# qiutang98/chord

Measured on AMD Instinct MI355X. Metric: Gtri/s into 4K 64-bit visbuffer, higher is better.
Workload: dtype f32+u64; 1 GPU; street_4k_hzb; scene_triangles_lod0=2799616, objects=352, hzb=True, cull=flat, parallelism=single

## Files before the change

chord_amd/csrc/device_layer.h:

```cpp
#pragma once

#include <hip/hip_runtime.h>
#include <cstddef>

#include <string>
#include <vector>

#include "chordvis.h"

#ifndef RASTER_PROFILE
#define RASTER_PROFILE 0
#endif
#ifndef RASTER_ABLATION
#define RASTER_ABLATION 0
#endif
#define CHORD_DEBUG_PROFILE_BITS (16u | 512u)
#define CHORD_DEBUG_ABLATION_BITS (1u | 2u | 32u | 64u | 128u | 256u | 1024u | 2048u | 4096u | 8192u | 16384u | 1048576u | 2097152u)

namespace chord {


struct DPrim {
    float    posMin[3]; uint32_t meshletBase;
    float    posMax[3]; uint32_t groupBase;
// ... 121 lines not shown
struct TriRecC {
    int32_t  X0, Y0;
    int16_t  dX1, dY1, dX2, dY2;
    float    d[3];
    uint32_t payload;
};
#define CHORD_REC_WIDE 0x80000000u
#define CHORD_REC_BLOCK 0xC0000000u
#define CHORD_REC_INDEX_MASK 0x3FFFFFFFu
#define CHORD_REC_MASKED 0xA0000000u
#define CHORD_REC_WIDE_INDEX 0x1FFFFFFFu
#define CHORD_BLOCK_WIN 16
struct ClipTri { uint32_t objectId, meshletId, slot, tri; };

#define CHORD_LIST_SHARDS 64u
#define CHORD_SHARD_STRIDE 16u
struct DeviceCounters {
    uint32_t triCount[CHORD_LIST_SHARDS * CHORD_SHARD_STRIDE];
    uint32_t triCountC[CHORD_LIST_SHARDS * CHORD_SHARD_STRIDE];
    uint32_t clipTriCount[2];
    uint32_t largeCount[2][CHORD_LIST_SHARDS * CHORD_SHARD_STRIDE];
    uint32_t overflow;
    uint32_t binPoolCount[2];
    uint32_t pad;
    uint32_t blockGranules[CHORD_LIST_SHARDS * CHORD_SHARD_STRIDE];
    uint32_t pad3[10];
    unsigned long long trisInstanceCulled, trisHzbVisible0, trisHzbVisible1, pad2;
};

#define CHORD_BIN_CHUNK_SHIFT 10
#define CHORD_BIN_CHUNK (1u << CHORD_BIN_CHUNK_SHIFT)
#define CHORD_BIN_MAX_CHUNKS_DEFAULT 240u
#define CHORD_BIN_MAX_CHUNKS_LIMIT 3072u
#define CHORD_TILE_MAX_SLICES 64u
#define CHORD_BIN_CHUNK_INVALID 0xFFFFFFFFu
#define CHORD_TILE_SLICE_SHIFT 11
#define CHORD_HOT_TILES 32u
#ifndef CHORD_TILE_SHIFT
#define CHORD_TILE_SHIFT 6
#endif
#define CHORD_TILE (1 << CHORD_TILE_SHIFT)
#define CHORD_MAX_TILES ((4096u >> CHORD_TILE_SHIFT) * (4096u >> CHORD_TILE_SHIFT))
#if CHORD_TILE_SHIFT == 6
#define CHORD_TILECOUNT_STRIDE 16u
#ifndef CHORD_BIN_CAP
#define CHORD_BIN_CAP 16384u
#endif
#else
#define CHORD_TILECOUNT_STRIDE 4u
#define CHORD_BIN_CAP 8192u
#endif
static_assert(CHORD_BIN_CAP <= (1u << 20), "tile x bin capacity is formed with a 24-bit multiply in 32 bits (bin_put)");
struct FrameState {
    DeviceCounters counters;
    uint32_t listCounts[8];
    uint32_t tileCount[2 * CHORD_MAX_TILES * CHORD_TILECOUNT_STRIDE];
};

static_assert(offsetof(FrameState, counters.trisInstanceCulled) % 64 == 0 && offsetof(FrameState, listCounts) == offsetof(FrameState, counters.trisInstanceCulled) + 32 &&
              offsetof(FrameState, tileCount) == offsetof(FrameState, listCounts) + 32, "triangle totals + list counts: one 64-byte line (frame_cull_fused_kernel)");

struct CmdList {
    uint32_t*     count = nullptr;
    ChordDrawCmd* cmds = nullptr;
    uint32_t      capacity = 0;
    ChordCountAndCmd handle() const { return ChordCountAndCmd{count, cmds, capacity}; }
};

struct HzbBuffers {
    ChordHZBDesc desc{};
    uint16_t* minTexels = nullptr;
    uint16_t* maxTexels = nullptr;
    uint32_t* validRange = nullptr;
    bool valid = false;
    bool uploaded = false;
    ChordHZB handle() const { return ChordHZB{desc, minTexels, maxTexels, validRange}; }
};

enum StampTag { S_FRAME_BEGIN = 0, S_CLEAR, S_CULL, S_HZBCULL, S_R_CLUSTER, S_R_CLIP, S_R_CHUNK, S_STAGE0_END,
                S_HZB0, S_STAGE1_END, S_HZBF, S_OTHER,
                S_EXCH_HZB, S_EXCH_VIS,
                S_EXCH_CULL,
                S_EXCH_FINAL };

}

struct ChordCtx {
    int device = 0;
    hipStream_t stream = nullptr;
    bool ownStream = false;
    std::string lastError;
    int numCUs = 256;

    bool sceneLoaded = false;
    uint32_t objectCount = 0, primCount = 0, materialCount = 0;
    uint32_t meshletCount = 0, groupCount = 0;
    uint32_t groupInstances = 0;
    uint32_t cmdCapacity = 0;
    uint64_t instTriangles = 0;
    chord::DPrim* dPrims = nullptr;
    chord::DGroup* dGroups = nullptr;
    chord::DMeshlet* dMeshlets = nullptr;
    uint32_t* dGroupIndices = nullptr;
    uint32_t* dMeshletData = nullptr;
    float* dPositions = nullptr;
    chord::DObjStatic* dObjStatic = nullptr;
// ... 195 lines not shown
```

chord_amd/csrc/kernels_raster.hip:

```cpp

#include "device_layer.h"
#include "device_math.h"

#include <algorithm>
#include <cstdlib>
#include <cstring>
#include <type_traits>

namespace chord {

#define GUARD_BAND 1024.0f
#define LDS_VERTS 256
#define TILE CHORD_TILE
#define TILE_SHIFT CHORD_TILE_SHIFT
#define TPITCH (TILE + 1)
#define SMALL_AREA 256
#define TC_STRIDE CHORD_TILECOUNT_STRIDE
#define TC_BLOCKS 1u
#define TC_TICKET 2u
#ifndef CHORD_MASKED_FUSED
#define CHORD_MASKED_FUSED 1
#endif
#define TC_MASKED 3u

struct RasterParams {
    const uint32_t* count; const ChordDrawCmd* cmds;
    uint32_t cmdCap;
    uint32_t* leftCount; ChordDrawCmd* leftCmds;
    const DObjFrame* objFrame; const DObjStatic* objStatic;
    const DMeshlet* meshlets; const uint32_t* meshletData; const float* positions;
    const DMaterial* materials; const uint8_t* texAlpha; const float* texcoords;
    unsigned long long* vis;
    float* depthOut;
    float W, H; int32_t Wi, Hi;
    ShardInfo shard;
    TriRec* tris; uint32_t triCap;
    TriRecC* trisC; uint32_t triCapC;
    uint32_t* tileCount; uint32_t* tileBins; uint32_t binCap; uint32_t tilesX, tilesY;
    uint32_t* binPool; uint32_t binPoolChunks; uint32_t* binPoolCount;
    unsigned long long* binChunkTab; uint32_t binStamp; uint32_t binMaxChunks;
    unsigned long long* blockPool; uint32_t blockCap;
    uint32_t blockForce;
    ClipTri* clipTris; uint32_t clipTriCap; uint32_t pass;
    uint32_t* largeList; uint32_t largeCap;
    DeviceCounters* counters;
    uint2* tileOrder;
    unsigned long long* tileSlabs;
    uint32_t hzbFused;
    ChordHZBDesc hzbDesc;
    uint16_t* hzbMinA;
    uint16_t* hzbMinB; uint16_t* hzbMaxB;
    uint16_t* hzbExA;
    uint16_t* hzbExB;
    uint32_t* tileRange;
    unsigned long long* tileClocks;
    unsigned long long* tilePhase;
    uint32_t depthOnly, depthClamp;
    float biasConst, biasSlope;
    uint32_t clearTiles;
    uint32_t* binHint;
    uint32_t* countHint;
    uint32_t slotHot;
    uint32_t* hotTiles;
    uint32_t tileSlots;
    uint32_t tileSplitMin, tileSliceLen;
    uint2* tileOrderNext;
    uint32_t orderAll;
    uint32_t orderKept;
    uint32_t* heavyHint;
    uint32_t debug;
};
#define ABL(p, flag) (RASTER_ABLATION && ((p).debug & (flag)) != 0u)
#define DBG_NO_PIXELS   1u
#define DBG_NO_BIN      2u
#define DBG_TILE_CLOCKS 16u
#define DBG_NO_OUT      128u
#define DBG_NO_HZB      256u
#define DBG_SETUP_CLOCKS 512u
#define DBG_NO_VIS_STORE 1024u
#define DBG_NO_SPLIT    2048u
#define DBG_NO_TINY     32u
#define DBG_TILE_EXIT   64u
#define DBG_NO_ENTRY    8192u
#define DBG_NO_BATCH    16384u
#define DBG_NO_UNITS    4096u
#define DBG_SKIP_LIGHT  1048576u
#define DBG_SKIP_HEAVY  2097152u

template <typename T>
__device__ __forceinline__ T scalar_load(const T* ptr)
{
    return *reinterpret_cast<const __attribute__((address_space(4))) T*>(reinterpret_cast<uintptr_t>(ptr));
}
__device__ __forceinline__ const RasterParams* kernel_args()
{
    unsigned long long kp = (unsigned long long)__builtin_amdgcn_kernarg_segment_ptr();
    asm volatile("" : "+s"(kp));
    return reinterpret_cast<const RasterParams*>(kp);
}

__device__ __forceinline__ uint32_t mbcnt64(unsigned long long m) { return __builtin_amdgcn_mbcnt_hi((uint32_t)(m >> 32), __builtin_amdgcn_mbcnt_lo((uint32_t)m, 0u)); }
__device__ __forceinline__ int32_t bcast(int32_t v, int src) { return __builtin_amdgcn_readlane(v, src); }
__device__ __forceinline__ uint32_t bcast(uint32_t v, int src) { return (uint32_t)__builtin_amdgcn_readlane((int)v, src); }
__device__ __forceinline__ float bcast(float v, int src) { return __int_as_float(__builtin_amdgcn_readlane(__float_as_int(v), src)); }

__device__ __forceinline__ bool owns_tile(const ShardInfo& s, int32_t tx, int32_t ty)
{
    if (s.ranks <= 1) return true;
    return shard_owns_tile(s, (uint32_t)tx, (uint32_t)ty);
}
__device__ __forceinline__ bool owns_rect(const ShardInfo& s, int32_t px0, int32_t py0, int32_t px1, int32_t py1)
{
    if (s.ranks <= 1) return true;
    return shard_owns_any_tile(s, (uint32_t)px0 >> TILE_SHIFT, (uint32_t)py0 >> TILE_SHIFT, (uint32_t)px1 >> TILE_SHIFT, (uint32_t)py1 >> TILE_SHIFT);
}

__device__ __forceinline__ bool in_fast_volume_xy(const f4& h)
{
    return h.w > 0.0f && (GUARD_BAND * h.w + h.x) >= 0.0f && (GUARD_BAND * h.w - h.x) >= 0.0f &&
           (GUARD_BAND * h.w + h.y) >= 0.0f && (GUARD_BAND * h.w - h.y) >= 0.0f;
}

// ... 71 lines not shown
    const float dzdx = ((float)(double)(a1 * 256) * invA) * e1 + ((float)(double)(a2 * 256) * invA) * e2;
    const float dzdy = ((float)(double)(b1 * 256) * invA) * e1 + ((float)(double)(b2 * 256) * invA) * e2;
    const float m = fmaxf(fabsf(dzdx), fabsf(dzdy));
    const float mz = fmaxf(fabsf(d[0]), fmaxf(fabsf(d[1]), fabsf(d[2])));
    const int32_t e = (int32_t)((__float_as_uint(mz) >> 23) & 0xFFu) - 23;
    const float r = (e > 0 && e < 255) ? __uint_as_float((uint32_t)e << 23) : 0.0f;
    return biasSlope * m + biasConst * r;
}

__device__ __forceinline__ void tri_setup_from_compact(TriSetup& ts, const TriRecC& r, int32_t Wi, int32_t Hi)
{
    ts.X[0] = r.X0; ts.Y[0] = r.Y0;
    ts.X[1] = r.X0 + r.dX1; ts.Y[1] = r.Y0 + r.dY1;
    ts.X[2] = r.X0 + r.dX2; ts.Y[2] = r.Y0 + r.dY2;
    ts.payload = r.payload;
    const int32_t area2 = (int32_t)r.dX1 * (int32_t)r.dY2 - (int32_t)r.dX2 * (int32_t)r.dY1;
    ts.s = area2 < 0 ? -1 : 1;
    ts.invA = 1.0f / (float)(area2 < 0 ? -area2 : area2);
    ts.d0 = r.d[0]; ts.e1 = r.d[1] - r.d[0]; ts.e2 = r.d[2] - r.d[0];
    const int32_t minX = min(ts.X[0], min(ts.X[1], ts.X[2])), maxX = max(ts.X[0], max(ts.X[1], ts.X[2]));
    const int32_t minY = min(ts.Y[0], min(ts.Y[1], ts.Y[2])), maxY = max(ts.Y[0], max(ts.Y[1], ts.Y[2]));
    ts.px0 = max(0, (minX + 127) >> 8);
    ts.py0 = max(0, (minY + 127) >> 8);
    ts.px1 = min(Wi - 1, (maxX - 128) >> 8);
    ts.py1 = min(Hi - 1, (maxY - 128) >> 8);
    ts.area = 0;
}

__device__ __forceinline__ void tri_setup_from_record(TriSetup& ts, const TriRec& r, int32_t Wi, int32_t Hi)
{
#pragma unroll
    for (int i = 0; i < 3; i++) { ts.X[i] = r.X[i]; ts.Y[i] = r.Y[i]; }
    ts.payload = r.payload;
    ts.s = (r.twoSided & 2u) ? -1 : 1;
    ts.invA = __uint_as_float(r.pad);
    ts.d0 = r.d[0]; ts.e1 = r.d[1] - r.d[0]; ts.e2 = r.d[2] - r.d[0];
    const int32_t minX = min(ts.X[0], min(ts.X[1], ts.X[2])), maxX = max(ts.X[0], max(ts.X[1], ts.X[2]));
    const int32_t minY = min(ts.Y[0], min(ts.Y[1], ts.Y[2])), maxY = max(ts.Y[0], max(ts.Y[1], ts.Y[2]));
    ts.px0 = max(0, (minX + 127) >> 8);
    ts.py0 = max(0, (minY + 127) >> 8);
    ts.px1 = min(Wi - 1, (maxX - 128) >> 8);
    ts.py1 = min(Hi - 1, (maxY - 128) >> 8);
    ts.area = 0;
}



struct RecordEmitParams {
    DeviceCounters* counters; ClipTri* clipTris; uint32_t clipTriCap; uint32_t pass;
    TriRec* tris; uint32_t triCap; TriRecC* trisC; uint32_t triCapC; uint32_t* largeList; uint32_t largeCap;
    uint32_t* tileCount; uint32_t* tileBins; uint32_t binCap; uint32_t tilesX;
    uint32_t* binPool; uint32_t binPoolChunks; uint32_t* binPoolCount;
    unsigned long long* binChunkTab; uint32_t binStamp; uint32_t binMaxChunks;
    ShardInfo shard;
};
__device__ __forceinline__ RecordEmitParams load_record_emit_params()
{
    const RasterParams* q = kernel_args();
    RecordEmitParams e;
    e.counters = scalar_load(&q->counters); e.clipTris = scalar_load(&q->clipTris); e.clipTriCap = scalar_load(&q->clipTriCap); e.pass = scalar_load(&q->pass);
    e.tris = scalar_load(&q->tris); e.triCap = scalar_load(&q->triCap); e.trisC = scalar_load(&q->trisC); e.triCapC = scalar_load(&q->triCapC);
    e.largeList = scalar_load(&q->largeList); e.largeCap = scalar_load(&q->largeCap);
    e.tileCount = scalar_load(&q->tileCount); e.tileBins = scalar_load(&q->tileBins); e.binCap = scalar_load(&q->binCap); e.tilesX = scalar_load(&q->tilesX);
    e.binPool = scalar_load(&q->binPool); e.binPoolChunks = scalar_load(&q->binPoolChunks); e.binPoolCount = scalar_load(&q->binPoolCount);
    e.binChunkTab = scalar_load(&q->binChunkTab); e.binStamp = scalar_load(&q->binStamp); e.binMaxChunks = scalar_load(&q->binMaxChunks);
    e.shard.ranks = scalar_load(&q->shard.ranks); e.shard.rank = scalar_load(&q->shard.rank); e.shard.slotsPerRank = 0u; e.shard.tilesX = 0u;
    e.shard.ownedRows = scalar_load(&q->shard.ownedRows); e.shard.tileSlot = nullptr;
    return e;
}

struct BinElect { int leader; uint32_t rank, group; };

__device__ __forceinline__ BinElect wave_bin_elect(bool has, uint32_t tile, uint32_t lane)
{
    BinElect e; e.leader = 0; e.rank = 0; e.group = 0;
    unsigned long long todo = __ballot(has);
    const unsigned long long lt = (1ull << lane) - 1ull;
    while (todo) {
        const int l = __ffsll((long long)todo) - 1;
        const uint32_t k = bcast(tile, l);
        const unsigned long long same = __ballot(has && tile == k);
        if (has && tile == k) { e.leader = l; e.rank = (uint32_t)__popcll(same & lt); e.group = (uint32_t)__popcll(same); }
        todo &= ~same;
    }
    return e;
}

__device__ __forceinline__ uint32_t bin_capacity(const RasterParams& p) { return p.binCap + p.binMaxChunks * CHORD_BIN_CHUNK; }

template <class P>
__device__ __forceinline__ void bin_alloc(const P& p, uint32_t tile, uint32_t slot)
{
#ifdef EXP_NO_CHUNKS
    return;
#endif
    if (slot < p.binCap) return;
    const uint32_t o = slot - p.binCap, j = o >> CHORD_BIN_CHUNK_SHIFT;
    if (j >= p.binMaxChunks || (o & (CHORD_BIN_CHUNK - 1u)) != 0u) return;
    uint32_t id = atomicAdd(p.binPoolCount, 1u);
    if (id >= p.binPoolChunks) { id = CHORD_BIN_CHUNK_INVALID; atomicOr(&p.counters->overflow, 1u); }
    __hip_atomic_store(p.binChunkTab + (__umul24(tile, p.binMaxChunks) + j), ((unsigned long long)p.binStamp << 32) | id,
                       __ATOMIC_RELAXED, __HIP_MEMORY_SCOPE_AGENT);
}

template <class P>
__device__ __forceinline__ void bin_put(const P& p, uint32_t tile, uint32_t slot, uint32_t gi)
{
#ifdef EXP_NO_CHUNKS
    slot &= p.binCap - 1u;
#endif
    if (slot < p.binCap) { p.tileBins[__umul24(tile, p.binCap) + slot] = gi; return; }
    const uint32_t o = slot - p.binCap, j = o >> CHORD_BIN_CHUNK_SHIFT;
    if (j >= p.binMaxChunks) { atomicOr(&p.counters->overflow, 1u); return; }
    const unsigned long long* ent = p.binChunkTab + (__umul24(tile, p.binMaxChunks) + j);
    const unsigned long long stamp = (unsigned long long)p.binStamp << 32;
    unsigned long long e = 0;
    uint32_t spins = 0;
    for (;;) {
        e = __hip_atomic_load(ent, __ATOMIC_RELAXED, __HIP_MEMORY_SCOPE_AGENT);
        if ((e & 0xFFFFFFFF00000000ull) == stamp) break;
        if (++spins > (1u << 20)) { atomicOr(&p.counters->overflow, 4u); return; }
        __builtin_amdgcn_s_sleep(4);
    }
    const uint32_t id = (uint32_t)e;
    if (id != CHORD_BIN_CHUNK_INVALID) p.binPool[((size_t)id << CHORD_BIN_CHUNK_SHIFT) + (o & (CHORD_BIN_CHUNK - 1u))] = gi;
}

__device__ __forceinline__ void bin_store(const RasterParams& p, uint32_t tile, uint32_t slot, uint32_t gi)
{
    bin_alloc(p, tile, slot);
    bin_put(p, tile, slot, gi);
}

struct BinTicket {
    uint32_t tileA[4], tileB[4], slotA[4], slotB[4];
    uint32_t has;
    uint32_t eA[4], eB[4];
};

template <class P>
__device__ __forceinline__ void wave_bin_issue(const P& p, bool emitA, const TriSetup& tsA, bool emitB, const TriSetup& tsB,
                                               uint32_t lane, BinTicket& k, const bool masked = false)
{
    auto tile_of = [&](const TriSetup& ts, int r, bool emit, uint32_t& tile) -> bool {
        const int32_t tx0 = ts.px0 >> TILE_SHIFT, tx1 = ts.px1 >> TILE_SHIFT, ty0 = ts.py0 >> TILE_SHIFT, ty1 = ts.py1 >> TILE_SHIFT;
// ... 474 lines not shown
                const uint32_t li = ebaseW + wSlots * (uint32_t)__popcll(ewA & lt);
                if (li + wSlots <= e.triCap) {
                    giA = listShard * e.triCap + li; write_record(&e.tris[giA], tsA, dA, twoSided, masked);
                    if (MASKED && masked) setup_emit_mask_ext(p, &e.tris[giA + 1u], triWord[0], uvA, lW, CHORD_MATFLAG_MATERIAL(hdr.matFlags), tsA.area);
                    giA |= (MASKED && masked) ? CHORD_REC_MASKED : CHORD_REC_WIDE; okA = true;
                } else atomicOr(&e.counters->overflow, 1u);
            }
            if (cpB) {
                const uint32_t li = ebaseC + (uint32_t)__popcll(ecA) + (uint32_t)__popcll(ecB & lt);
                if (li < e.triCapC) { giB = listShard * e.triCapC + li; write_record_c(&e.trisC[giB], tsB, dB); okB = true; }
                else atomicOr(&e.counters->overflow, 1u);
            } else if (kindB == K_EMIT) {
                const uint32_t li = ebaseW + wSlots * ((uint32_t)__popcll(ewA) + (uint32_t)__popcll(ewB & lt));
                if (li + wSlots <= e.triCap) {
                    giB = listShard * e.triCap + li; write_record(&e.tris[giB], tsB, dB, twoSided, masked);
                    if (MASKED && masked) setup_emit_mask_ext(p, &e.tris[giB + 1u], triWord[1], uvB, lW, CHORD_MATFLAG_MATERIAL(hdr.matFlags), tsB.area);
                    giB |= (MASKED && masked) ? CHORD_REC_MASKED : CHORD_REC_WIDE; okB = true;
                } else atomicOr(&e.counters->overflow, 1u);
            }
            if (emA | emB) wave_bin_commit(e, ticket, okA, giA, okB, giB);
            if (lgA && okA) {
                const uint32_t k = lbase + (uint32_t)__popcll(lmA & lt);
                if (k < e.largeCap) e.largeList[(size_t)listShard * e.largeCap + k] = giA & CHORD_REC_WIDE_INDEX; else atomicOr(&e.counters->overflow, 1u);
            }
            if (lgB && okB) {
                const uint32_t k = lbase + (uint32_t)__popcll(lmA) + (uint32_t)__popcll(lmB & lt);
                if (k < e.largeCap) e.largeList[(size_t)listShard * e.largeCap + k] = giB & CHORD_REC_WIDE_INDEX; else atomicOr(&e.counters->overflow, 1u);
            }
            }
        }
        __builtin_amdgcn_fence(__ATOMIC_RELEASE, "wavefront");
        __builtin_amdgcn_wave_barrier();
        hdr = hdrN;
        hdrN = load_header(c + 2u * stride);
        t0 = nt0; t1 = nt1;
        pax = nax; pay = nay; paz = naz; pbx = nbx; pby = nby; pbz = nbz;
        SPHASE(4);
    }
    if (sprof && lane == 0u) {
        const uint32_t w = blockIdx.x * 4u + wave;
        if (w < CHORD_MAX_TILES * 8u / 5u) for (int i = 0; i < 5; i++) p.tilePhase[(size_t)w * 5u + i] = sph[i];
    }
#undef SPHASE
}

struct SetupHeader { uint32_t objectId, meshletId, slot, V, T, dataOffset, vertexBase, matFlags; };

struct BlockEmitParams {
    uint32_t* tileCount; uint32_t* tileBins; uint32_t binCap;
    uint32_t* binPool; uint32_t binPoolChunks; uint32_t* binPoolCount;
    unsigned long long* binChunkTab; uint32_t binStamp; uint32_t binMaxChunks;
    unsigned long long* blockPool; uint32_t blockCap;
    DeviceCounters* counters;
};
__device__ __forceinline__ BlockEmitParams load_block_emit_params()
{
    const RasterParams* q = kernel_args();
    BlockEmitParams e;
    e.tileCount = scalar_load(&q->tileCount); e.tileBins = scalar_load(&q->tileBins); e.binCap = scalar_load(&q->binCap);
    e.binPool = scalar_load(&q->binPool); e.binPoolChunks = scalar_load(&q->binPoolChunks); e.binPoolCount = scalar_load(&q->binPoolCount);
    e.binChunkTab = scalar_load(&q->binChunkTab); e.binStamp = scalar_load(&q->binStamp); e.binMaxChunks = scalar_load(&q->binMaxChunks);
    e.blockPool = scalar_load(&q->blockPool); e.blockCap = scalar_load(&q->blockCap);
    e.counters = scalar_load(&q->counters);
    return e;
}

#define WAVE_LDS_SYNC() do { __builtin_amdgcn_fence(__ATOMIC_RELEASE, "wavefront"); __builtin_amdgcn_wave_barrier(); __builtin_amdgcn_fence(__ATOMIC_ACQUIRE, "wavefront"); } while (0)

__device__ __forceinline__ int classify_triangle(const RasterParams& p, uint32_t t, uint32_t T, uint32_t packedIdx, bool twoSided, bool allFast,
                                                 const float* lX, const float* lY, const float* lW, const float* lU, const float* lV, const float* lD,
                                                 const int32_t* lSX, const int32_t* lSY, uint32_t& boxX, uint32_t& boxY, bool& narrow)
{
    boxX = 0u; boxY = 0u; narrow = false;
    if (t >= T) return K_NONE;
    const uint32_t i0 = packedIdx & 0xFFu, i1 = (packedIdx >> 8) & 0xFFu, i2 = (packedIdx >> 16) & 0xFFu;
    const float w0 = lW[i0], w1 = lW[i1], w2 = lW[i2];
    bool culled = false;
    if (!twoSided) {
        const float x0 = lX[i0], y0 = lY[i0], x1 = lX[i1], y1 = lY[i1], x2 = lX[i2], y2 = lY[i2];
        const float det = (x0 * (y1 * w2 - w1 * y2) - y0 * (x1 * w2 - w1 * x2)) + w0 * (x1 * y2 - y1 * x2);
        culled = det <= 0.0f;
    }
    culled = culled || (w0 <= 0.0f && w1 <= 0.0f && w2 <= 0.0f);
    const float u0 = lU[i0], v0 = lV[i0], u1 = lU[i1], v1 = lV[i1], u2 = lU[i2], v2 = lV[i2];
    const float maxU = fmaxf(u0, fmaxf(u1, u2)), maxV = fmaxf(v0, fmaxf(v1, v2));
    const float minU = fminf(u0, fminf(u1, u2)), minV = fminf(v0, fminf(v1, v2));
    culled = culled || ((minU >= 1.0f || minV >= 1.0f) || (maxU <= 0.0f || maxV <= 0.0f));
    culled = culled || (rintf(minU * p.W) == rintf(maxU * p.W) || rintf(minV * p.H) == rintf(maxV * p.H));
    if (culled) return K_NONE;
    if (!allFast) { const float d0 = lD[i0], d1 = lD[i1], d2 = lD[i2]; if (d0 != d0 || d1 != d1 || d2 != d2) return K_CLIP; }
    const int32_t X0 = lSX[i0], Y0 = lSY[i0], X1 = lSX[i1], Y1 = lSY[i1], X2 = lSX[i2], Y2 = lSY[i2];
    const int32_t minX = min(X0, min(X1, X2)), maxX = max(X0, max(X1, X2));
    const int32_t minY = min(Y0, min(Y1, Y2)), maxY = max(Y0, max(Y1, Y2));
    if (maxX - minX > (1 << 14) || maxY - minY > (1 << 14)) return K_EMIT;
    narrow = true;
    const int32_t area2 = __mul24(X1 - X0, Y2 - Y0) - __mul24(X2 - X0, Y1 - Y0);
    if (area2 == 0 || (!twoSided && area2 > 0)) return K_NONE;
    const int32_t px0 = max(0, (minX + 127) >> 8), py0 = max(0, (minY + 127) >> 8);
    const int32_t px1 = min(p.Wi - 1, (maxX - 128) >> 8), py1 = min(p.Hi - 1, (maxY - 128) >> 8);
    if (px1 < px0 || py1 < py0) return K_NONE;
    boxX = (uint32_t)px0 | ((uint32_t)px1 << 16); boxY = (uint32_t)py0 | ((uint32_t)py1 << 16);
    return K_EMIT;
}

__device__ __forceinline__ void resolve_entry(const RasterParams& p, uint32_t entry, uint32_t boxX, uint32_t boxY, uint32_t slot,
                                              const int32_t* lSX, const int32_t* lSY, const float* lD, unsigned long long* win,
                                              int32_t bx0, int32_t by0)
{
    const uint32_t i0 = entry & 0xFFu, i1 = (entry >> 8) & 0xFFu, i2 = (entry >> 16) & 0xFFu, t = entry >> 24;
    TriSetup ts;
    ts.X[0] = lSX[i0]; ts.Y[0] = lSY[i0];
    ts.X[1] = lSX[i1]; ts.Y[1] = lSY[i1];
    ts.X[2] = lSX[i2]; ts.Y[2] = lSY[i2];
    const int32_t dx1 = ts.X[1] - ts.X[0], dy1 = ts.Y[1] - ts.Y[0], dx2 = ts.X[2] - ts.X[0], dy2 = ts.Y[2] - ts.Y[0];
    const int32_t area2 = __mul24(dx1, dy2) - __mul24(dx2, dy1);
    const int32_t area = area2 < 0 ? -area2 : area2;
// ... 1282 lines not shown
        if (lane != 0u) merge_block_word(tile, A[j].x, 2u * lane - 1u, H[j], R[j]);                                       \
        if (2u * lane < N[j]) merge_block_word(tile, A[j].y, 2u * lane, H[j], R[j]);                                      \
    }                                                                                                                     \
    _Pragma("unroll") for (int j = 0; j < 4; j++)                                                                         \
        for (uint32_t g = lane + 64u; 2u * g <= N[j]; g += 64u) {                                                         \
            const ulonglong2 v = SRC[j][g];                                                                               \
            merge_block_word(tile, v.x, 2u * g - 1u, H[j], R[j]);                                                         \
            if (2u * g < N[j]) merge_block_word(tile, v.y, 2u * g, H[j], R[j]);                                           \
        }
    if (!todo) return;
#ifndef MB_GROUPS
#define MB_GROUPS 2
#endif
#if MB_GROUPS == 3
    uint32_t hA[4], rA[4], nA[4], hB[4], rB[4], nB[4], hC[4], rC[4], nC[4];
    const ulonglong2* srcA[4];
    const ulonglong2* srcB[4];
    const ulonglong2* srcC[4];
    ulonglong2 aA[4], aB[4], aC[4];
    MB_PICK(hA, rA, nA, srcA) MB_LOAD(aA, nA, srcA)
    MB_PICK(hB, rB, nB, srcB) MB_LOAD(aB, nB, srcB)
    MB_PICK(hC, rC, nC, srcC) MB_LOAD(aC, nC, srcC)
    do {
        MB_MERGE(aA, hA, rA, nA, srcA) MB_PICK(hA, rA, nA, srcA) MB_LOAD(aA, nA, srcA)
        MB_MERGE(aB, hB, rB, nB, srcB) MB_PICK(hB, rB, nB, srcB) MB_LOAD(aB, nB, srcB)
        MB_MERGE(aC, hC, rC, nC, srcC) MB_PICK(hC, rC, nC, srcC) MB_LOAD(aC, nC, srcC)
    } while ((nA[0] | nB[0] | nC[0]) != 0u);
#else
    uint32_t hA[4], rA[4], nA[4], hB[4], rB[4], nB[4];
    const ulonglong2* srcA[4];
    const ulonglong2* srcB[4];
    ulonglong2 aA[4], aB[4];
    MB_PICK(hA, rA, nA, srcA)
    MB_LOAD(aA, nA, srcA)
    for (;;) {
        const bool moreB = todo != 0ull;
        if (moreB) { MB_PICK(hB, rB, nB, srcB) MB_LOAD(aB, nB, srcB) }
        MB_MERGE(aA, hA, rA, nA, srcA)
        if (!moreB) break;
        const bool moreA = todo != 0ull;
        if (moreA) { MB_PICK(hA, rA, nA, srcA) MB_LOAD(aA, nA, srcA) }
        MB_MERGE(aB, hB, rB, nB, srcB)
        if (!moreA) break;
    }
#endif
#undef MB_PICK
#undef MB_LOAD
#undef MB_MERGE
}

#ifndef TILE_DEEP_FETCH
#define TILE_DEEP_FETCH 0
#endif
#ifndef TILE_MIN_BLOCKS
#define TILE_MIN_BLOCKS 4
#endif
template <bool SH, bool MASKED, bool DEPTH>
__global__ __launch_bounds__(TB, TILE_MIN_BLOCKS) void raster_tile_kernel(RasterParams p)
{
    __shared__ __align__(16) unsigned long long tile[TILE * TPITCH];
    __shared__ EntrySoA prm;
    __shared__ uint32_t unitList[TILE_UNIT_CAP];
    __shared__ uint32_t offs[16];
    __shared__ uint32_t waveSums[2][TB / 64];
    __shared__ uint32_t chunkTab[64];
    __shared__ uint32_t sTicket;
    if (ABL(p, DBG_TILE_EXIT) && !p.clearTiles) return;
#define TILE_SKEW (scalar_load(&kernel_args()->tileOrderNext) != nullptr ? 1u : 0u)
#define wgs (gridDim.x - TILE_SKEW)
    const uint32_t tilesAll = p.tilesX * p.tilesY;
    const uint32_t wg0 = blockIdx.x - (p.tileOrderNext != nullptr ? 1u : 0u);
    if (p.tileOrderNext && blockIdx.x == 0u) {
#if TILE_MAKE_NEXT
        tile_order_next_part(kernel_args());
#endif
        return;
    }
    const bool direct = p.orderKept == 2u;
    uint2 firstItem = make_uint2(wg0, 0u);
    uint32_t active = tilesAll;
    if (!direct) { firstItem = p.tileOrder[1u + min(wg0, tilesAll - 1u)]; active = p.tileOrder[0].x; }
    for (uint32_t oiw = wg0; (oiw & 0x7FFFFFFFu) < active; oiw = ((oiw & 0x7FFFFFFFu) + wgs) | 0x80000000u) {
    const uint32_t oi = oiw & 0x7FFFFFFFu;
    uint32_t tix = threadIdx.x;
    asm volatile("" : "+v"(tix));
    const uint2 itemCount = (oiw >> 31) == 0u ? firstItem : (direct ? make_uint2(oi, 0u) : p.tileOrder[1u + oi]);
    const uint32_t item = itemCount.x;
    const uint32_t tileId = item & 0xFFFu, slice = (item >> 12) & 0x3FFu, slices = (item >> 22) + 1u;
    const uint32_t* bin = p.tileBins + (size_t)tileId * p.binCap;
    const bool entryThread = TILE_BATCH == TB || tix < TILE_BATCH;
    uint32_t countWord = itemCount.y, wordSpec = 0xFFFFFFFFu;
    if (p.orderKept) {
        if (entryThread) wordSpec = bin[tix];
        const unsigned long long cnt = scalar_load(reinterpret_cast<const unsigned long long*>(&p.tileCount[(size_t)tileId * TC_STRIDE]));
        countWord = min((uint32_t)cnt, bin_capacity(p)) | ((uint32_t)(cnt >> 32) ? 0x80000000u : 0u);
    }
    const uint32_t nAll = countWord & 0x3FFFFFFFu;
    if (ABL(p, DBG_SKIP_LIGHT) && nAll < 64u) continue;
    if (ABL(p, DBG_SKIP_HEAVY) && nAll >= 64u) continue;
    if (direct) {
        if (p.heavyHint && tix == 0u) {
            if (nAll > p.tileSplitMin) p.heavyHint[0] = p.binStamp;
            if (oi == 0u) p.heavyHint[*p.count > TILE_DIRECT_MAX_CLUSTERS ? 0 : 2] = p.binStamp;
        }
        if (nAll == 0u) continue;
    }
    if (p.orderAll && !p.clearTiles && nAll == 0u) continue;
    const bool hasBlocks = (countWord >> 31) != 0u;
    const bool preloaded = !CHORD_MASKED_FUSED && p.clearTiles && (countWord & 0x40000000u) != 0u;
    const int32_t tinyArea = nAll >= TINY_DENSE_MIN ? TINY_AREA_DENSE : TINY_AREA;
    const uint32_t per = slices > 1u ? ((nAll + slices - 1u) / slices + TB - 1u) & ~(TB - 1u) : nAll;
    const uint32_t lo = slices > 1u ? min(nAll, slice * per) : 0u;
    const uint32_t n = ABL(p, DBG_NO_BATCH) ? lo : (slices > 1u ? min(nAll, lo + per) : nAll);
    const bool prof = RASTER_PROFILE && (p.debug & DBG_TILE_CLOCKS) != 0;
    const unsigned long long t0 = prof ? wall_clock64() : 0ull;
    unsigned long long ph[6] = {0, 0, 0, 0, 0, 0}, tp = t0;
    uint32_t cUnits = 0, cUnitIters = 0, cTiny = 0, cTinyIters = 0;
    unsigned long long bw[6] = {0, 0, 0, 0, 0, 0};
#define PHASE(i) do { if (prof) { const unsigned long long ta = wall_clock64(); __syncthreads(); const unsigned long long tn = wall_clock64(); bw[i] += tn - ta; ph[i] += tn - tp; tp = tn; } } while (0)
    const int32_t ox = (int32_t)(tileId % p.tilesX) * TILE, oy = (int32_t)(tileId / p.tilesX) * TILE;
    const int32_t tw = min(TILE, p.Wi - ox), th = min(TILE, p.Hi - oy);
    const bool noPixels = ABL(p, DBG_NO_PIXELS);
    auto slot_of_tile = [&]() -> uint32_t { return SH ? __builtin_amdgcn_readfirstlane(scalar_load(&kernel_args()->shard.tileSlot)[tileId]) : 0u; };
    auto vis_base = [&]() -> uint32_t { return SH ? slot_of_tile() << (2 * TILE_SHIFT) : (uint32_t)oy * (uint32_t)p.Wi + (uint32_t)ox; };
    const uint32_t visPitch = SH ? (uint32_t)TILE : (uint32_t)p.Wi;

    const bool early = n <= p.binCap && !hasBlocks;
    const uint32_t k0 = lo + tix;
    const uint32_t word0 = (early && entryThread && k0 < n) ? ((p.orderKept && slices == 1u) ? wordSpec : bin[k0]) : 0xFFFFFFFFu;

    const bool rmw = (p.hzbFused && !p.clearTiles) || preloaded;
    const bool mergeSlices = slices > 1u && (p.clearTiles || rmw);
    if (!(rmw && !mergeSlices)) {
        static_assert((TILE * TPITCH) % 2 == 0, "whole 16-byte words");
        for (uint32_t i = tix; i < TILE * TPITCH / 2; i += TB) reinterpret_cast<ulonglong2*>(tile)[i] = make_ulonglong2(0ull, 0ull);
    } else
    for (uint32_t i = tix, visBase = vis_base(); i < TILE * TILE / 2; i += TB) {
        const int32_t ly = (int32_t)(i >> (TILE_SHIFT - 1)), lx = (int32_t)(i & (TILE / 2 - 1)) * 2;
        ulonglong2 v = make_ulonglong2(0ull, 0ull);
// ... 441 lines not shown
    p.tileBins = c->dTileBins + (size_t)pass * tiles * c->binCap; p.binCap = c->binCap;
    p.binPool = c->dBinPool + (size_t)pass * c->binPoolChunks * CHORD_BIN_CHUNK; p.binPoolChunks = c->binPoolChunks;
    p.binPoolCount = &c->dCounters->binPoolCount[pass];
    p.binChunkTab = c->dBinChunkTab + (size_t)pass * tiles * c->binMaxChunks; p.binMaxChunks = c->binMaxChunks;
    p.binStamp = ++c->rasterSerial;
    p.tilesX = c->tilesX; p.tilesY = c->tilesY;
    p.clipTris = c->dClipTris + (size_t)pass * (c->clipTriCap / 2); p.clipTriCap = c->clipTriCap / 2; p.pass = pass;
    p.largeList = c->dLargeList + (size_t)pass * (c->largeCap / 2); p.largeCap = c->largeCap / 2 / CHORD_LIST_SHARDS;
    p.counters = c->dCounters;
    p.clearTiles = clearTiles ? 1u : 0u;
    p.depthOnly = c->depthOnly ? 1u : 0u; p.depthClamp = c->depthClamp ? 1u : 0u;
    p.biasConst = c->depthBiasConst; p.biasSlope = c->depthBiasSlope;
    p.debug = c->debugFlags;
    p.tileClocks = c->dTileClocks + (size_t)pass * CHORD_MAX_TILES;
    p.tileOrder = reinterpret_cast<uint2*>(c->dTileOrder); p.tileSlabs = c->dTileSlabs;
    p.tilePhase = c->dTileClocks + (size_t)2 * CHORD_MAX_TILES + (size_t)pass * CHORD_MAX_TILES * 8;

    if (!c->inFrame || c->rasterCalls >= 2) {
        LR_HIP(hipMemsetAsync(p.tileCount, 0, sizeof(uint32_t) * TC_STRIDE * tiles, c->stream));
        LR_HIP(hipMemsetAsync(&c->dCounters->clipTriCount[pass], 0, sizeof(uint32_t), c->stream));
        LR_HIP(hipMemsetAsync(c->dCounters->largeCount[pass], 0, sizeof(c->dCounters->largeCount[pass]), c->stream));
        LR_HIP(hipMemsetAsync(&c->dCounters->binPoolCount[pass], 0, sizeof(uint32_t), c->stream));
        if (!c->inFrame) { LR_HIP(hipMemsetAsync(c->dCounters->triCount, 0, sizeof(c->dCounters->triCount), c->stream));
                           LR_HIP(hipMemsetAsync(c->dCounters->triCountC, 0, sizeof(c->dCounters->triCountC), c->stream));
                           LR_HIP(hipMemsetAsync(c->dCounters->blockGranules, 0, sizeof(c->dCounters->blockGranules), c->stream)); }
    }

    const uint64_t rankPixels = (uint64_t)c->width * c->height / (c->shard.ranks > 1 ? c->shard.ranks : 1u);
    const bool maybeDense = p.blockCap != 0u && (p.blockForce != 0u || (uint64_t)in.capacity * 16ull >= rankPixels);
    p.leftCount = nullptr; p.leftCmds = nullptr;
    p.binHint = nullptr; p.countHint = nullptr;
    p.slotHot = (c->debugFlags & DBG_FORCE_HOT) ? 64u : SLOT_HOT;
    {
        static const int forced = [] { const char* e = getenv("CHORDVIS_TILE_SLOTS"); return e ? atoi(e) : -1; }();
        p.tileSlots = forced >= 0 ? (uint32_t)forced : c->shard.ranks > 1 ? (uint32_t)c->numCUs * (CHORD_TILE_SHIFT == 6 ? 2u : 6u) : 0u;
        static const int splitMin = [] { const char* e = getenv("CHORDVIS_TILE_SPLIT_MIN"); return e ? atoi(e) : -1; }();
        static const int sliceLen = [] { const char* e = getenv("CHORDVIS_TILE_SLICE"); return e ? atoi(e) : -1; }();
        p.tileSplitMin = splitMin > 0 ? (uint32_t)splitMin : TILE_SPLIT_MIN;
        p.tileSliceLen = sliceLen >= 512 ? ((uint32_t)sliceLen + 511u) & ~511u : TILE_SLICE;
    }
    p.hotTiles = c->dHotTiles ? c->dHotTiles + (size_t)pass * (1u + CHORD_HOT_TILES) : nullptr;
    bool blocksWorthLaunching = maybeDense;
    if (maybeDense && c->dBinHint) {
        p.countHint = c->dBinHint + 2 + pass;
        const uint32_t last = c->hBinHint[2 + pass];
        if (p.blockForce == 0u && last != 0xFFFFFFFFu && (uint64_t)last * 32ull < rankPixels) blocksWorthLaunching = false;
    }
    if (blocksWorthLaunching) {
        if (c->dBinHint) p.binHint = c->dBinHint + pass;
        if (!c->dLeftCmds) LR_HIP(hipMalloc((void**)&c->dLeftCmds, sizeof(ChordDrawCmd) * (size_t)c->cmdCapacity));
        p.leftCount = c->dCounts + 6 + pass; p.leftCmds = c->dLeftCmds;
        if (!c->inFrame || c->rasterCalls >= 2) LR_HIP(hipMemsetAsync(p.leftCount, 0, sizeof(uint32_t), c->stream));
    }
    uint32_t blocks = (in.capacity + 3u) / 4u;
#ifndef SETUP_GRID_MULT
#define SETUP_GRID_MULT 1u
#endif
    const uint32_t maxBlocks = (uint32_t)c->numCUs * SETUP_MIN_WAVES * SETUP_GRID_MULT;
    if (blocks > maxBlocks) blocks = maxBlocks;
    if (blocks < 1) blocks = 1;
    const bool sh = c->shard.ranks > 1;
    stamp(c, S_HZBCULL);
    if (blocksWorthLaunching) {
        const uint32_t bb = std::max(1u, std::min((in.capacity + 3u) / 4u, (uint32_t)c->numCUs * BLOCKS_MIN_WAVES));
        const bool hot = (c->hBinHint && c->hBinHint[pass] >= SLOT_HOT) || (c->debugFlags & DBG_FORCE_HOT);
        if (hot) CHORD_LAUNCH(c, raster_setup_blocks_kernel<true>, dim3(bb), dim3(256), 0, c->stream, p);
        else     CHORD_LAUNCH(c, raster_setup_blocks_kernel<false>, dim3(bb), dim3(256), 0, c->stream, p);
    }
    if (c->anyMasked) CHORD_LAUNCH(c, raster_setup_kernel<true>, dim3(blocks), dim3(256), 0, c->stream, p);
    else              CHORD_LAUNCH(c, raster_setup_kernel<false>, dim3(blocks), dim3(256), 0, c->stream, p);
    stamp(c, S_R_CLUSTER);
    CHORD_LAUNCH(c, raster_clip_and_bin_large_kernel, dim3(CLIP_BLOCKS + (uint32_t)c->numCUs * 4u), dim3(256), 0, c->stream, p);
    p.orderKept = 0u;
    p.heavyHint = nullptr;
    bool makeOrder = true;
    static const bool directOn = [] { const char* e = getenv("CHORDVIS_TILE_DIRECT"); return !e || atoi(e) != 0; }();
    const bool laterOk = c->inFrame && !clearTiles && p.hzbFused && !c->depthOnly && CHORD_MASKED_FUSED && c->dBinHint && !(c->debugFlags & ~(DBG_NO_BLOCKS | DBG_FORCE_BLOCKS | DBG_FORCE_HOT | 524288u));
    if (laterOk) p.heavyHint = c->dBinHint + 4 + pass;
    if (TILE_DIRECT && directOn && laterOk) {
        const uint32_t heavySeen = c->hBinHint[4 + pass], lightSeen = c->hBinHint[6 + pass];
        if (lightSeen != 0u && (heavySeen == 0u || (int32_t)(lightSeen - heavySeen) > 0)) {
            p.orderKept = 2u; makeOrder = false;
        }
    }
    p.orderAll = 0u; p.tileOrderNext = nullptr;
    static const bool keepLaterOn = [] { const char* e = getenv("CHORDVIS_TILE_KEEP_LATER"); return !e || atoi(e) != 0; }();
    static const bool nextOn = [] { const char* e = getenv("CHORDVIS_TILE_NEXT"); return !e || atoi(e) != 0; }();
    const bool keepOk = TILE_ORDER_KEEP && c->orderKeepFrames && CHORD_MASKED_FUSED && c->inFrame && !c->depthOnly && !(c->debugFlags & ~524288u);
    int slot = -1;
    if (keepOk && clearTiles && pass == 0u && c->dTileOrderKeep) slot = 0;
    else if (keepOk && keepLaterOn && laterOk && pass == 1u && c->dTileOrderKeep1) slot = 1;
    if (slot >= 0) {
        uint32_t& age = slot ? c->orderAge1 : c->orderAge;
        uint2* buf = reinterpret_cast<uint2*>(slot ? c->dTileOrderKeep1 : c->dTileOrderKeep);
        const size_t half = (size_t)1 + c->tileItemCap;
        p.orderAll = slot ? 1u : 0u;
        if (nextOn && p.orderKept == 2u) {
            age = 0xFFFFFFFFu; p.orderAll = 0u;
        } else if (nextOn) {
            uint32_t& flip = c->orderFlip[slot];
            p.tileOrder = buf + flip * half; p.tileOrderNext = buf + (flip ^ 1u) * half;
            if (age != 0xFFFFFFFFu) { p.orderKept = 1u; makeOrder = false; }
            age = 0u; flip ^= 1u;
        } else if (p.orderKept != 2u) {
            p.tileOrder = buf;
            if (age < c->orderKeepFrames) { age++; p.orderKept = 1u; makeOrder = false; }
            else age = 0u;
        } else p.orderAll = 0u;
    }
    if (makeOrder) CHORD_LAUNCH(c, raster_tile_order_kernel, dim3(1), dim3(1024), 0, c->stream, p);
#if !CHORD_MASKED_FUSED
    if (c->anyMasked) {
        const uint32_t items = tiles;
        if (c->depthClamp && !sh) CHORD_LAUNCH(c, (raster_masked_tile_kernel<false, true>), dim3(items), dim3(TB), 0, c->stream, p);
        else if (sh)              CHORD_LAUNCH(c, (raster_masked_tile_kernel<true, false>), dim3(items), dim3(TB), 0, c->stream, p);
        else                      CHORD_LAUNCH(c, (raster_masked_tile_kernel<false, false>), dim3(items), dim3(TB), 0, c->stream, p);
    }
#endif
    stamp(c, S_R_CLIP);
    const uint32_t tileBlocks = (p.tileOrderNext ? 1u : 0u) + ((clearTiles || p.orderKept == 2u || p.orderAll) ? ((sh && clearTiles) ? min(tiles, max(c->shard.slotsPerRank, p.tileSlots + p.tileSlots / 2u)) : tiles) : min(tiles, (uint32_t)c->numCUs * (CHORD_TILE_SHIFT == 6 ? 2u : 6u)));
#if CHORD_MASKED_FUSED
    if (c->anyMasked) {
        if (c->depthClamp && !sh) CHORD_LAUNCH(c, (raster_tile_kernel<false, true, true>), dim3(tileBlocks), dim3(TB), 0, c->stream, p);
        else if (sh)              CHORD_LAUNCH(c, (raster_tile_kernel<true, true, false>), dim3(tileBlocks), dim3(TB), 0, c->stream, p);
        else                      CHORD_LAUNCH(c, (raster_tile_kernel<false, true, false>), dim3(tileBlocks), dim3(TB), 0, c->stream, p);
    } else
#endif
    if (c->depthClamp && !sh) {
        CHORD_LAUNCH(c, (raster_tile_kernel<false, false, true>), dim3(tileBlocks), dim3(TB), 0, c->stream, p);
    } else {
        if (sh) CHORD_LAUNCH(c, (raster_tile_kernel<true, false, false>), dim3(tileBlocks), dim3(TB), 0, c->stream, p);
        else    CHORD_LAUNCH(c, (raster_tile_kernel<false, false, false>), dim3(tileBlocks), dim3(TB), 0, c->stream, p);
    }
    stamp(c, S_R_CHUNK);
    c->rasterCalls++;
    return hipSuccess;
#undef LR_HIP
}

}
```

Before: 3.229 Gtri/s.

## Track touched tiles in a bitmask and launch tile raster only over occupied tiles

Binning now sets a per-tile bit in a new touched bitmask when a tile gets its first bin entry. In the direct tile-order path, the raster tile kernel uses a wave-wide prefix popcount select to map each workgroup onto occupied tiles, and the grid is capped at a CU-scaled slot count instead of one block per tile. This is meant to avoid launching and scanning empty tiles in the later HZB pass. In exchange it adds an atomicOr per new tile, a memset per pass, and select logic at tile-kernel entry. The direct-path decision is moved earlier so the mask can be set up before the setup and binning kernels run.

```diff
diff --git a/chord_amd/csrc/device_layer.h b/chord_amd/csrc/device_layer.h
--- a/chord_amd/csrc/device_layer.h
+++ b/chord_amd/csrc/device_layer.h
@@ -197,6 +197,7 @@
 #endif
 static_assert(CHORD_BIN_CAP <= (1u << 20), "tile x bin capacity is formed with a 24-bit multiply in 32 bits (bin_put)");
 struct FrameState {
+    uint32_t tileTouched[2 * CHORD_MAX_TILES / 32];
     DeviceCounters counters;
     uint32_t listCounts[8];
     uint32_t tileCount[2 * CHORD_MAX_TILES * CHORD_TILECOUNT_STRIDE];
diff --git a/chord_amd/csrc/kernels_raster.hip b/chord_amd/csrc/kernels_raster.hip
--- a/chord_amd/csrc/kernels_raster.hip
+++ b/chord_amd/csrc/kernels_raster.hip
@@ -68,6 +68,7 @@
     uint32_t orderAll;
     uint32_t orderKept;
     uint32_t* heavyHint;
+    uint32_t* tileTouched;
     uint32_t debug;
 };
 #define ABL(p, flag) (RASTER_ABLATION && ((p).debug & (flag)) != 0u)
@@ -245,6 +246,7 @@
     uint32_t* tileCount; uint32_t* tileBins; uint32_t binCap; uint32_t tilesX;
     uint32_t* binPool; uint32_t binPoolChunks; uint32_t* binPoolCount;
     unsigned long long* binChunkTab; uint32_t binStamp; uint32_t binMaxChunks;
+    uint32_t* tileTouched;
     ShardInfo shard;
 };
 __device__ __forceinline__ RecordEmitParams load_record_emit_params()
@@ -257,6 +259,7 @@
     e.tileCount = scalar_load(&q->tileCount); e.tileBins = scalar_load(&q->tileBins); e.binCap = scalar_load(&q->binCap); e.tilesX = scalar_load(&q->tilesX);
     e.binPool = scalar_load(&q->binPool); e.binPoolChunks = scalar_load(&q->binPoolChunks); e.binPoolCount = scalar_load(&q->binPoolCount);
     e.binChunkTab = scalar_load(&q->binChunkTab); e.binStamp = scalar_load(&q->binStamp); e.binMaxChunks = scalar_load(&q->binMaxChunks);
+    e.tileTouched = scalar_load(&q->tileTouched);
     e.shard.ranks = scalar_load(&q->shard.ranks); e.shard.rank = scalar_load(&q->shard.rank); e.shard.slotsPerRank = 0u; e.shard.tilesX = 0u;
     e.shard.ownedRows = scalar_load(&q->shard.ownedRows); e.shard.tileSlot = nullptr;
     return e;
@@ -284,6 +287,7 @@
 template <class P>
 __device__ __forceinline__ void bin_alloc(const P& p, uint32_t tile, uint32_t slot)
 {
+    if (slot == 0u && p.tileTouched) atomicOr(&p.tileTouched[tile >> 5], 1u << (tile & 31u));
 #ifdef EXP_NO_CHUNKS
     return;
 #endif
@@ -864,6 +868,7 @@
     unsigned long long* binChunkTab; uint32_t binStamp; uint32_t binMaxChunks;
     unsigned long long* blockPool; uint32_t blockCap;
     DeviceCounters* counters;
+    uint32_t* tileTouched;
 };
 __device__ __forceinline__ BlockEmitParams load_block_emit_params()
 {
@@ -874,6 +879,7 @@
     e.binChunkTab = scalar_load(&q->binChunkTab); e.binStamp = scalar_load(&q->binStamp); e.binMaxChunks = scalar_load(&q->binMaxChunks);
     e.blockPool = scalar_load(&q->blockPool); e.blockCap = scalar_load(&q->blockCap);
     e.counters = scalar_load(&q->counters);
+    e.tileTouched = scalar_load(&q->tileTouched);
     return e;
 }
 
@@ -2262,6 +2268,31 @@
 #ifndef TILE_DEEP_FETCH
 #define TILE_DEEP_FETCH 0
 #endif
+__device__ __forceinline__ uint32_t touched_tile(const uint32_t* __restrict__ mask, uint32_t k, uint32_t g, uint32_t& total, uint32_t& tail)
+{
+    const uint32_t lane = threadIdx.x & 63u;
+    const uint2 w = reinterpret_cast<const uint2*>(mask)[lane];
+    const uint32_t c = (uint32_t)(__popc(w.x) + __popc(w.y));
+    uint32_t incl = c;
+#pragma unroll
+    for (uint32_t d = 1u; d < 64u; d <<= 1) { const uint32_t t = __shfl_up(incl, d, 64); if (lane >= d) incl += t; }
+    total = bcast(incl, 63);
+    auto select = [&](uint32_t j) -> uint32_t {
+        uint32_t r = j - (incl - c), m = w.x, pos = 0u;
+        const uint32_t nLo = (uint32_t)__popc(w.x);
+        if (r >= nLo) { r -= nLo; m = w.y; pos = 32u; }
+#pragma unroll
+        for (uint32_t s = 16u; s != 0u; s >>= 1) {
+            const uint32_t n = (uint32_t)__popc(m & ((1u << s) - 1u));
+            if (r >= n) { r -= n; m >>= s; pos += s; }
+        }
+        const unsigned long long holder = __ballot(incl - c <= j && j < incl);
+        return holder ? bcast(lane * 64u + pos, (int)__ffsll((long long)holder) - 1) : 0u;
+    };
+    tail = select(g - 1u) + 1u;
+    return select(k);
+}
+
 #ifndef TILE_MIN_BLOCKS
 #define TILE_MIN_BLOCKS 4
 #endif
@@ -2290,11 +2321,17 @@
     uint2 firstItem = make_uint2(wg0, 0u);
     uint32_t active = tilesAll;
     if (!direct) { firstItem = p.tileOrder[1u + min(wg0, tilesAll - 1u)]; active = p.tileOrder[0].x; }
+    else if (p.tileTouched) {
+        uint32_t touched, tail;
+        firstItem.x = touched_tile(p.tileTouched, wg0, gridDim.x, touched, tail);
+        active = touched > gridDim.x ? gridDim.x + tilesAll - tail : touched;
+        if (active == 0u && wg0 == 0u && threadIdx.x == 0u && p.heavyHint) p.heavyHint[*p.count > TILE_DIRECT_MAX_CLUSTERS ? 0 : 2] = p.binStamp;
+    }
     for (uint32_t oiw = wg0; (oiw & 0x7FFFFFFFu) < active; oiw = ((oiw & 0x7FFFFFFFu) + wgs) | 0x80000000u) {
     const uint32_t oi = oiw & 0x7FFFFFFFu;
     uint32_t tix = threadIdx.x;
     asm volatile("" : "+v"(tix));
-    const uint2 itemCount = (oiw >> 31) == 0u ? firstItem : (direct ? make_uint2(oi, 0u) : p.tileOrder[1u + oi]);
+    const uint2 itemCount = (oiw >> 31) == 0u ? firstItem : (direct ? make_uint2(oi + tilesAll - active, 0u) : p.tileOrder[1u + oi]);
     const uint32_t item = itemCount.x;
     const uint32_t tileId = item & 0xFFFu, slice = (item >> 12) & 0x3FFu, slices = (item >> 22) + 1u;
     const uint32_t* bin = p.tileBins + (size_t)tileId * p.binCap;
@@ -2842,6 +2879,23 @@
         p.leftCount = c->dCounts + 6 + pass; p.leftCmds = c->dLeftCmds;
         if (!c->inFrame || c->rasterCalls >= 2) LR_HIP(hipMemsetAsync(p.leftCount, 0, sizeof(uint32_t), c->stream));
     }
+    p.orderKept = 0u;
+    p.heavyHint = nullptr;
+    static const bool directOn = [] { const char* e = getenv("CHORDVIS_TILE_DIRECT"); return !e || atoi(e) != 0; }();
+    const bool laterOk = c->inFrame && !clearTiles && p.hzbFused && !c->depthOnly && CHORD_MASKED_FUSED && c->dBinHint && !(c->debugFlags & ~(DBG_NO_BLOCKS | DBG_FORCE_BLOCKS | DBG_FORCE_HOT | 524288u));
+    if (laterOk) p.heavyHint = c->dBinHint + 4 + pass;
+    if (TILE_DIRECT && directOn && laterOk) {
+        const uint32_t heavySeen = c->hBinHint[4 + pass], lightSeen = c->hBinHint[6 + pass];
+        if (lightSeen != 0u && (heavySeen == 0u || (int32_t)(lightSeen - heavySeen) > 0)) {
+            p.orderKept = 2u;
+        }
+    }
+    static const int touchedEnv = [] { const char* e = getenv("CHORDVIS_TILE_TOUCHED"); return e ? atoi(e) : 1; }();
+    p.tileTouched = nullptr;
+    if (p.orderKept == 2u && touchedEnv != 0 && c->shard.ranks <= 1 && tiles <= 64u * 64u) {
+        p.tileTouched = c->dFrameState->tileTouched + (size_t)pass * (CHORD_MAX_TILES / 32u);
+        if (!c->inFrame || c->rasterCalls >= 2) LR_HIP(hipMemsetAsync(p.tileTouched, 0, sizeof(uint32_t) * ((tiles + 31u) / 32u), c->stream));
+    }
     uint32_t blocks = (in.capacity + 3u) / 4u;
 #ifndef SETUP_GRID_MULT
 #define SETUP_GRID_MULT 1u
@@ -2861,18 +2915,7 @@
     else              CHORD_LAUNCH(c, raster_setup_kernel<false>, dim3(blocks), dim3(256), 0, c->stream, p);
     stamp(c, S_R_CLUSTER);
     CHORD_LAUNCH(c, raster_clip_and_bin_large_kernel, dim3(CLIP_BLOCKS + (uint32_t)c->numCUs * 4u), dim3(256), 0, c->stream, p);
-    p.orderKept = 0u;
-    p.heavyHint = nullptr;
-    bool makeOrder = true;
-    static const bool directOn = [] { const char* e = getenv("CHORDVIS_TILE_DIRECT"); return !e || atoi(e) != 0; }();
-    const bool laterOk = c->inFrame && !clearTiles && p.hzbFused && !c->depthOnly && CHORD_MASKED_FUSED && c->dBinHint && !(c->debugFlags & ~(DBG_NO_BLOCKS | DBG_FORCE_BLOCKS | DBG_FORCE_HOT | 524288u));
-    if (laterOk) p.heavyHint = c->dBinHint + 4 + pass;
-    if (TILE_DIRECT && directOn && laterOk) {
-        const uint32_t heavySeen = c->hBinHint[4 + pass], lightSeen = c->hBinHint[6 + pass];
-        if (lightSeen != 0u && (heavySeen == 0u || (int32_t)(lightSeen - heavySeen) > 0)) {
-            p.orderKept = 2u; makeOrder = false;
-        }
-    }
+    bool makeOrder = p.orderKept != 2u;
     p.orderAll = 0u; p.tileOrderNext = nullptr;
     static const bool keepLaterOn = [] { const char* e = getenv("CHORDVIS_TILE_KEEP_LATER"); return !e || atoi(e) != 0; }();
     static const bool nextOn = [] { const char* e = getenv("CHORDVIS_TILE_NEXT"); return !e || atoi(e) != 0; }();
@@ -2908,7 +2951,9 @@
     }
 #endif
     stamp(c, S_R_CLIP);
-    const uint32_t tileBlocks = (p.tileOrderNext ? 1u : 0u) + ((clearTiles || p.orderKept == 2u || p.orderAll) ? ((sh && clearTiles) ? min(tiles, max(c->shard.slotsPerRank, p.tileSlots + p.tileSlots / 2u)) : tiles) : min(tiles, (uint32_t)c->numCUs * (CHORD_TILE_SHIFT == 6 ? 2u : 6u)));
+    const uint32_t slots = (uint32_t)c->numCUs * (CHORD_TILE_SHIFT == 6 ? 2u : 6u);
+    const uint32_t tileBlocks = (p.tileOrderNext ? 1u : 0u) + ((clearTiles || (p.orderKept == 2u && !p.tileTouched) || p.orderAll) ? ((sh && clearTiles) ? min(tiles, max(c->shard.slotsPerRank, p.tileSlots + p.tileSlots / 2u)) : tiles)
+                                                               : min(tiles, p.tileTouched && touchedEnv > 1 ? (uint32_t)touchedEnv : slots));
 #if CHORD_MASKED_FUSED
     if (c->anyMasked) {
         if (c->depthClamp && !sh) CHORD_LAUNCH(c, (raster_tile_kernel<false, true, true>), dim3(tileBlocks), dim3(TB), 0, c->stream, p);
```

Result: faster. 3.279 Gtri/s, median of 6 (+1.5%).
